# tohtsky/myFM

Measured on AMD Instinct MI355X. Metric: Gibbs iterations/sec (rank=32), higher is better.
Workload: dtype f64

## Files before the change

myfm_amd/csrc/mfm_hip.hip:

```cpp
#include <algorithm>
#include <cerrno>
#include <chrono>
#include <cmath>
#include <cstdio>
#include <cstring>
#include <map>
#include <memory>
#include <mutex>
#include <string>
#include <thread>
#include <type_traits>
#include <vector>

#include <fcntl.h>
#include <sys/file.h>
#include <sys/stat.h>
#include <unistd.h>

#include <hipcub/hipcub.hpp>

#include "mfm_common.hpp"
#include "mfm_kernels.hpp"
#include "mfm_plan.hpp"
#include "mfm_res_plan.hpp"
// ... 68 lines not shown
    d.claimed += want;
    return true;
  }
  void release(int device, int n) {
    if (n <= 0) return;
    std::lock_guard<std::mutex> g(m);
    Dev &d = dev[key_of(device)];
    d.claimed = std::max(0, d.claimed - n);
    if (d.claimed == 0 && d.lock_fd >= 0) {
      ::flock(d.lock_fd, LOCK_UN);
      ::close(d.lock_fd);
      d.lock_fd = -1;
    }
  }
};
}

struct mfm_ctx;
namespace mfm {
static void materialize_e(::mfm_ctx *c);
enum class EWhere : uint8_t { Rows, Slots, SlotsWithSums, Cell, Dropped };
enum class VPath : uint8_t { Deferred, Generic, QFree, Split, SplitFused, TwoField, ShardedSplit, ShardedTwoField, Cell };
enum class ResState : uint8_t { Off, Refused, AwaitingPeers, Live };
}
using namespace mfm;

struct mfm_ctx {
  int device = 0;
  hipStream_t stream = nullptr;
  bool own_stream = false;
  std::string err;
  bool finalized = false;

  HostCsr hX;
  bool main_set = false, hX_valid = false;
  const HostCsr &host_main() {
    if (main_set && !hX_valid) {
      hX = X.download();
      hX_valid = true;
    }
    return hX;
  }
  std::vector<double> hy;
  struct HostBlock {
    HostCsr X;
    std::unique_ptr<int32_t[]> map;
  };
  std::vector<HostBlock> hblocks;
  std::vector<int32_t> hgroup;
  std::vector<int32_t> hlevels;
  int32_t G = 0;

  int64_t N = 0, D0 = 0, D = 0;
  int K = 0, KS = 0;
  DevSparse X;
  StepPlan plan_V, plan_W;
  LongScratch ls;
  Comm comm;
  int64_t row_offset = 0;
  std::vector<std::unique_ptr<DevBlock>> blocks;
  DevBuf<double> y;
  DevBuf<double2> eq_;
  double2 *eq_raw() const { return eq_.p; }
  double2 *eq_rows() {
    mfm::materialize_e(this);
    return eq_.p;
  }
  EWhere e_where = EWhere::Rows;
  bool e_slot_order() const { return e_where == EWhere::Slots || e_where == EWhere::SlotsWithSums; }
  struct ResidentE {
    bool load_slots, no_store;
  };
  ResidentE e_for_resident(bool with_w, int f_begin, int f_end) const {
    return {e_slot_order(), with_w && e_recomputable && e_is_residual && f_begin == 0 && f_end == K};
  }
  void e_left_by_resident(const ResidentE &r) { e_where = r.no_store ? EWhere::Dropped : EWhere::Slots; }
  DevBuf<int32_t> group;
  DevBuf<int32_t> feat_sorted;
  DevBuf<int64_t> group_ptr;

  double w0 = 0;
  DevBuf<double> w, V, Vt;

  DevBuf<double> z;
  DevBuf<double> lam, mu;
  DevBuf<double2> red_partial;
  DevBuf<double2> red_out;
  DevBuf<double> scratch_n;
  DevBuf<double2> gs_partial;
  DevBuf<double2> hs_out;
  DevBuf<double> hs_mu;
  int gs_chunks = 1;
  DevBuf<double> ec, qc;
  VPath v_path = VPath::Generic;
  bool two_field() const { return v_path == VPath::TwoField || v_path == VPath::ShardedTwoField; }
  ResPlan res;
  ResState res_state = ResState::Off;
  bool resident_V() const { return res_state == ResState::Live; }
  std::vector<DevBuf<int32_t>> pre_maps;
  bool e_recomputable = false;
  bool e_is_residual = false;
  int res_plan_cus = 0;
  void ensure_main_plans();
  CellPlan cell;
  bool cell_w = false;
  int q_stale_factor = -1;
  BlockOverflow gather_overflow;
  DevBuf<double> wv_pack, zw_host;
  DevBuf<double> hyp, hyp_in, hyp_ng;
  std::vector<double> hyp_ng_host;
  hipEvent_t hyp_ev = nullptr;
  const double *w0_dev = nullptr;
  std::vector<double> hs_stage;
  bool res_fills_device = false;
  int res_claim = 0;
  DevBuf<double> sync_mask;
  PinnedRing ring;
  double2 *h_red = nullptr;
  size_t h_red_cap = 0;
  Timing timing;

  struct RngEngine {
    bool seeded = false, programmed = false;
    hipStream_t stream = nullptr;
    DevBuf<RngState> state, state_next;
    DevBuf<uint32_t> raw;
    DevBuf<uint32_t> jump;
    uint64_t need_gen = 0;
    int par_wgs = 1;
    int par_blocks = 0;
    DevBuf<uint32_t> starts;
    uint64_t mask = 0, need = 0;
    DevBuf<RngOp> ops;
    int n_ops = 0;
    int64_t n_hv = 0, n_zw = 0, n_zv = 0;
    struct Slot {
      DevBuf<double> hv, zw, zv;
      double *h_hv = nullptr;
      hipEvent_t ready = nullptr, free_ev = nullptr;
      bool free_valid = false;
    } slot[3];
    static constexpr int N_SLOTS = 3;
    hipEvent_t gate = nullptr;
    int pending_slot = -1, pending_op = 0;
    bool latent_pending = false;
    hipEvent_t latent_ev = nullptr;
    DevBuf<uint32_t> host_win;
    int64_t produced = 0, acquired = 0;
    int current = -1;
    std::vector<RngOp> h_ops;
    DevBuf<double> cand;
    DevBuf<unsigned long long> masks;
    DevBuf<int> counts;
    DevBuf<NormScratch> nscratch;
    static constexpr int64_t WIDE_COUNT = 262144;
    static int64_t attempts_for(int64_t count) {
      double a = (double)count * (4.0 / 3.14159265358979) * 1.01 + 8.0 * std::sqrt((double)count + 1.0) + 4096.0;
      int64_t n = (int64_t)a;
      return (n + NORM_CHUNK - 1) / NORM_CHUNK * NORM_CHUNK;
    }
    ~RngEngine() {
      for (auto &sl : slot) {
        if (sl.h_hv) (void)hipHostFree(sl.h_hv);
        if (sl.ready) (void)hipEventDestroy(sl.ready);
        if (sl.free_ev) (void)hipEventDestroy(sl.free_ev);
      }
      if (gate) (void)hipEventDestroy(gate);
      if (latent_ev) (void)hipEventDestroy(latent_ev);
      if (stream) (void)hipStreamDestroy(stream);
    }
  } rng;

  std::unique_ptr<LatentEngine> latent;
  LatentStats latent_stats;
  DevBuf<int32_t> latent_order;

  struct OGroup {
    int n_class = 0;
    int64_t n_rows = 0;
    DevBuf<int32_t> rows;
  };
  std::vector<std::unique_ptr<OGroup>> ogroups;
  int opartial_cmax = 0;
  DevBuf<double> oacc;

  DevBuf<double> opartial;

  ~mfm_ctx() {
    drop_resident();
    if (h_red) (void)hipHostFree(h_red);
    if (own_stream && stream) (void)hipStreamDestroy(stream);
  }
  void use_device() { MFM_HIP_CHECK(hipSetDevice(device)); }
  void drop_resident() {
    for (void *m : res.peer_mapped) (void)hipIpcCloseMemHandle(m);
    res.peer_mapped.clear();
    res_state = ResState::Off;
    res.peers_model = false;
    if (res_claim) ResidentBudget::get().release(device, res_claim);
    res_claim = 0;
    res_fills_device = false;
  }
  void check_coresident(int flag) {
    if (flag == 0) return;
    (void)hipMemsetAsync(ls.error.p, 0, sizeof(int), stream);
    (void)hipStreamSynchronize(stream);
    const bool had = resident_V();
    drop_resident();
    throw Error(MFM_ERR_RUNTIME,
                std::string("co-resident workgroups timed out waiting for each other (long-column sweep / conflict-batched chain / "
                            "resident latent sweep): the state of this fit is invalid") +
                    (flag == 2 ? " [a peer rank's sums did not arrive inside the row-sharded persistent sweep]" : "") +
                    (had ? "; the persistent sweep is switched off for this context" : ""));
  }
  void sync_and_check() {
    if (!ls.error.p) {
      MFM_HIP_CHECK(hipStreamSynchronize(stream));
      return;
    }
    double2 *h = readback(1);
    *(int *)h = 0;
    MFM_HIP_CHECK(hipMemcpyAsync(h, ls.error.p, sizeof(int), hipMemcpyDeviceToHost, stream));
    MFM_HIP_CHECK(hipStreamSynchronize(stream));
    check_coresident(*(const int *)h);
  }
  void need_final() const {
    if (!finalized) throw Error(MFM_ERR_RUNTIME, "mfm_finalize has not been called");
  }
  double2 *readback(size_t n) {
    if (h_red_cap < n) {
      if (h_red) MFM_HIP_CHECK(hipHostFree(h_red));
      h_red = nullptr;
      MFM_HIP_CHECK(hipHostMalloc((void **)&h_red, n * sizeof(double2), hipHostMallocDefault));
      h_red_cap = n;
    }
    return h_red;
  }
};

#define MFM_TRY(ctx) \
  try {              \
    (ctx)->use_device();
#define MFM_CATCH(ctx)                 \
  return MFM_OK;                       \
  }                                    \
  catch (const mfm::Error &ex) {       \
    (ctx)->err = ex.what();            \
    return ex.code;                    \
  }                                    \
  catch (const std::bad_alloc &) {     \
    (ctx)->err = "host out of memory"; \
    return MFM_ERR_RUNTIME;            \
  }                                    \
  catch (const std::exception &ex) {   \
    (ctx)->err = ex.what();            \
    return MFM_ERR_RUNTIME;            \
  }

namespace mfm {

static void fill_gather_args(std::vector<std::unique_ptr<DevBlock>> &blocks, BlockGatherArgs &g, BlockOverflow &ov, PinnedRing &ring,
                             hipStream_t s) {
  std::memset(&g, 0, sizeof(g));
  g.n_blocks = (int)blocks.size();
  std::vector<const int32_t *> xm;
  std::vector<const double *> xr;
  std::vector<int> xs;
  for (size_t b = 0; b < blocks.size(); b++) {
    const int32_t *m = blocks[b]->map.p;
    const double *r = blocks[b]->qc.p ? blocks[b]->qc.p : blocks[b]->rec.p;
    const int st = blocks[b]->qc.p ? 1 : BLOCK_REC;
    if (b < (size_t)MAX_BLOCKS) {
      g.map[b] = m;
      g.rec[b] = r;
      g.stride[b] = st;
    } else {
      xm.push_back(m);
      xr.push_back(r);
      xs.push_back(st);
    }
  }
  BlockOverflow::put(ov.map, xm, ring, s);
  BlockOverflow::put(ov.p0, xr, ring, s);
  BlockOverflow::put(ov.stride, xs, ring, s);
  g.xmap = ov.map.p;
  g.xrec = ov.p0.p;
  g.xstride = ov.stride.p;
}

static bool qbuild_by_rows(const mfm_ctx *c) { return c->X.avg_row_nnz <= 16.0; }
static void launch_qbuild(mfm_ctx *c, const double *vf, DevBlock *pending = nullptr) {
  if (c->N == 0) return;
  hipStream_t s = c->stream;
  BlockGatherArgs g;
  fill_gather_args(c->blocks, g, const_cast<mfm_ctx *>(c)->gather_overflow, const_cast<mfm_ctx *>(c)->ring, s);
  TimedLaunch t(c->timing, s, KC_QBUILD, 12.0 * c->X.nnz + 8.0 * c->N + 8.0 * c->D0 + 12.0 * c->N * g.n_blocks);
  if (qbuild_by_rows(c)) {
    const bool ell = c->X.ell_width >= 0;
    dim3 grid(cdiv(c->N, WG)), block(WG);
#define MFM_QB(U, E) \
  hipLaunchKernelGGL((k_qbuild_rows<U, E>), grid, block, 0, s, c->X.rowptr.p, c->X.colidx.p, c->X.rval.p, vf, c->eq_rows(), c->N, \
                     (int)c->X.ell_width, g, pending ? pending->map.p : (const int32_t *)nullptr,                          \
                     pending ? pending->q_saved.p : (const double2 *)nullptr)
    if (c->X.unit) {
      if (ell) MFM_QB(true, true); else MFM_QB(true, false);
    } else {
      if (ell) MFM_QB(false, true); else MFM_QB(false, false);
// ... 1750 lines not shown
    a.r_val = c->X.rval.p;
    a.r_ell = (int)c->X.ell_width;
    a.state = c->ec.p;
    if (c->v_path != VPath::QFree) {
      a.state2 = c->qc.p;
      a.aos = c->eq_rows();
    }
    return a;
  };
  const bool unit = c->X.unit;
  switch (c->v_path) {
    case VPath::QFree:
      hipLaunchKernelGGL(k_e_pack, dim3(cdiv(c->N, 256)), dim3(256), 0, s, c->eq_rows(), c->ec.p, c->N);
      for (int f = f_begin; f < f_end; f++) run_plan_qfree(s, c->timing, c->plan_V, args(f), c->ls, kcv, unit);
      hipLaunchKernelGGL(k_e_unpack, dim3(cdiv(c->N, 256)), dim3(256), 0, s, c->eq_rows(), c->ec.p, c->N);
      break;
    case VPath::ShardedTwoField:
    case VPath::ShardedSplit: {
      if (c->v_path == VPath::ShardedTwoField) {
        if (unit)
          run_sweep_mf<true>(s, c->timing, c->plan_V, args, f_begin, f_end, c->ls, kcv, &c->comm);
        else
          run_sweep_mf<false>(s, c->timing, c->plan_V, args, f_begin, f_end, c->ls, kcv, &c->comm);
      } else if (c->plan_V.steps.size() > 2) {
        if (unit)
          run_sweep_soa_multi<true>(s, c->timing, c->plan_V, args, f_begin, f_end, c->ls, kcv, &c->comm);
        else
          run_sweep_soa_multi<false>(s, c->timing, c->plan_V, args, f_begin, f_end, c->ls, kcv, &c->comm);
      } else if (unit) {
        run_sweep_soa_sharded<true>(s, c->timing, c->plan_V, args, f_begin, f_end, c->ls, kcv, c->comm);
      } else {
        run_sweep_soa_sharded<false>(s, c->timing, c->plan_V, args, f_begin, f_end, c->ls, kcv, c->comm);
      }
      sync_model_sharded(c, false, f_begin, f_end);
      break;
    }
    case VPath::TwoField:
    case VPath::SplitFused:
    case VPath::Split:
      if (c->v_path == VPath::TwoField) {
        if (unit)
          run_sweep_mf<true>(s, c->timing, c->plan_V, args, f_begin, f_end, c->ls, kcv);
        else
          run_sweep_mf<false>(s, c->timing, c->plan_V, args, f_begin, f_end, c->ls, kcv);
      } else if (unit)
        run_sweep_soa<true>(s, c->timing, c->plan_V, args, f_begin, f_end, c->ls, kcv, c->v_path == VPath::SplitFused);
      else
        run_sweep_soa<false>(s, c->timing, c->plan_V, args, f_begin, f_end, c->ls, kcv, c->v_path == VPath::SplitFused);
      if (!c->plan_V.steps.back().par.tiled)
        hipLaunchKernelGGL(k_e_unpack, dim3(cdiv(c->N, 256)), dim3(256), 0, s, c->eq_rows(), c->ec.p, c->N);
      break;
    case VPath::Cell:
      run_sweep_cell(c, f_begin, f_end, zbase, alpha);
      return MFM_OK;
    case VPath::Generic:
    case VPath::Deferred:
      sweep_V_generic(c, f_begin, f_end, zbase, alpha, kcv);
      return MFM_OK;
  }
  c->q_stale_factor = f_end - 1;
  MFM_HIP_CHECK(hipGetLastError());
  MFM_CATCH(ctx)
}

int mfm_update_e_regression(mfm_ctx *ctx) {
  MFM_TRY(ctx)
  ctx->need_final();
  score_train(ctx, true);
  MFM_CATCH(ctx)
}

int mfm_score_train(mfm_ctx *ctx) {
  MFM_TRY(ctx)
  ctx->need_final();
  score_train(ctx, false);
  MFM_CATCH(ctx)
}

int mfm_rng_seed_mt19937(mfm_ctx *ctx, const uint32_t *state624, int32_t position) {
  MFM_TRY(ctx)
  auto &r = ctx->rng;
  if (position < 0 || position > MT_N) throw Error(MFM_ERR_INVALID, "mt19937 position out of range");
  if (!r.stream) {
    int lo = 0, hi = 0;
    MFM_HIP_CHECK(hipDeviceGetStreamPriorityRange(&lo, &hi));
    MFM_HIP_CHECK(hipStreamCreateWithPriority(&r.stream, hipStreamNonBlocking, hi));
  }
  MFM_HIP_CHECK(hipStreamSynchronize(r.stream));
  RngState h;
  std::memset(&h, 0, sizeof(h));
  h.mt_pos = position;
  std::memcpy(h.mt, state624, sizeof(uint32_t) * MT_N);
  r.state.alloc(1);
  MFM_HIP_CHECK(hipMemcpy(r.state.p, &h, sizeof(h), hipMemcpyHostToDevice));
  r.seeded = true;
  r.produced = r.acquired = 0;
  r.current = -1;
  r.pending_slot = -1;
  for (auto &sl : r.slot) sl.free_valid = false;
  MFM_CATCH(ctx)
}

int mfm_rng_set_program(mfm_ctx *ctx, const mfm_rng_op *ops, int32_t n_ops) {
  MFM_TRY(ctx)
  auto &r = ctx->rng;
  if (!r.seeded) throw Error(MFM_ERR_RUNTIME, "mfm_rng_seed_mt19937 has not been called");
  if (r.produced != r.acquired) throw Error(MFM_ERR_RUNTIME, "cannot change the draw program while a set is in flight");
  MFM_HIP_CHECK(hipStreamSynchronize(r.stream));
  std::vector<RngOp> h((size_t)n_ops);
  int64_t n_dest[3] = {0, 0, 0};
  double normals = 0, gammas = 0;
  int n_normal_ops = 0;
  int64_t latent_rows = 0;
  int n_kept = 0;
  for (int k = 0; k < n_ops; k++) {
    const mfm_rng_op &o = ops[k];
    if (o.kind == MFM_RNG_LATENT) {
      if (o.count < 0) throw Error(MFM_ERR_INVALID, "bad rng op");
      latent_rows += o.count;
      continue;
    }
    const int i = n_kept++;
    if (o.kind != MFM_RNG_NORMALS && o.kind != MFM_RNG_GAMMA) throw Error(MFM_ERR_INVALID, "bad rng op kind");
    if (o.dest < 0 || o.dest > 2 || o.count < 0 || o.offset < 0) throw Error(MFM_ERR_INVALID, "bad rng op");
    if (o.kind == MFM_RNG_GAMMA && !(o.shape > 0)) throw Error(MFM_ERR_INVALID, "gamma shape must be positive");
    h[i].kind = o.kind;
    h[i].dest = o.dest;
    h[i].count = o.kind == MFM_RNG_GAMMA ? 1 : o.count;
    h[i].offset = o.offset;
    h[i].shape = o.shape;
    n_dest[o.dest] = std::max(n_dest[o.dest], o.offset + h[i].count);
    if (o.kind == MFM_RNG_GAMMA)
      gammas += 1;
    else {
      normals += (double)o.count;
      n_normal_ops++;
    }
  }
  h.resize((size_t)n_kept);
  n_ops = n_kept;
  r.n_hv = n_dest[0];
  r.n_zw = n_dest[1];
  r.n_zv = n_dest[2];
  r.ops.upload(h);
  r.h_ops = h;
  r.n_ops = n_ops;
  {
    int64_t amax = 0;
    for (auto &o : h)
      if (o.kind == MFM_RNG_NORMALS && o.count > 16384) amax = std::max(amax, mfm_ctx::RngEngine::attempts_for(o.count));
    r.cand.alloc((size_t)std::max<int64_t>(amax, 1));
    r.masks.alloc((size_t)std::max<int64_t>(amax / 64, 1));
    r.counts.alloc((size_t)std::max<int64_t>(amax / NORM_CHUNK, 1));
    r.nscratch.alloc(1);
  }
  const double per_normal = 4.0 * 4.0 / 3.14159265358979;
  r.need = (uint64_t)(normals * per_normal * 1.02 + 6.0 * 2.4 * std::sqrt(normals + 1.0) + gammas * 4096.0 +
                      4.0 * RNG_ATT * RNG_CONSUME_THREADS * (n_normal_ops + 1) + 65536.0);
  if (latent_rows > 0) r.need += (uint64_t)(4.0 * (1.6 * (double)latent_rows + 6.0 * std::sqrt((double)latent_rows) + 1024.0));
  for (auto &o : h)
    if (o.kind == MFM_RNG_NORMALS && o.count > 16384)
      r.need += (uint64_t)(4 * (mfm_ctx::RngEngine::attempts_for(o.count) - (int64_t)((double)o.count * 1.2732)));
  r.par_wgs = 1;
  r.need_gen = r.need;
  {
    const int64_t blocks1 = (int64_t)(r.need / MT_N) + 2;
    if (blocks1 > MT_PAR_BLOCKS) {
      r.need_gen = r.need * (uint64_t)(latent_rows > (1 << 22) ? 2 : mt_gen_batch((double)r.need));
      const int64_t blocks = (int64_t)(r.need_gen / MT_N) + 2;
      if (r.par_blocks <= 0) r.par_blocks = mt_par_blocks_for(blocks);
      const int wgs = (int)((blocks + r.par_blocks - 1) / r.par_blocks);
      std::vector<uint32_t> tab;
      if (mtjump::JumpCache::inst().get(r.par_blocks, wgs - 1, tab)) {
        r.jump.upload(tab);
        r.state_next.alloc(1);
        r.par_wgs = wgs;
        r.starts.alloc((size_t)wgs * MT_N);
        MFM_HIP_CHECK(hipFuncSetAttribute((const void *)k_mt_generate_par<0>, hipFuncAttributeMaxDynamicSharedMemorySize,
                                          (int)((MT_JUMP_SPAN * MT_N + 2 * (MT_N + 1)) * sizeof(uint32_t))));
        MFM_HIP_CHECK(hipFuncSetAttribute((const void *)k_mt_generate_par<1>, hipFuncAttributeMaxDynamicSharedMemorySize,
                                          (int)((MT_JUMP_SPAN * MT_N + 2 * (MT_N + 1)) * sizeof(uint32_t))));
      }
    }
  }
  uint64_t cap = 1;
  while (cap < r.need_gen + r.need + 2 * MT_N) cap <<= 1;
  r.raw.alloc((size_t)cap);
  r.mask = cap - 1;
  for (auto &sl : r.slot) {
    sl.hv.alloc((size_t)std::max<int64_t>(r.n_hv, 1));
    sl.zw.alloc((size_t)std::max<int64_t>(r.n_zw, 1));
    sl.zv.alloc((size_t)std::max<int64_t>(r.n_zv, 1));
    if (sl.h_hv) MFM_HIP_CHECK(hipHostFree(sl.h_hv));
    sl.h_hv = nullptr;
    MFM_HIP_CHECK(hipHostMalloc((void **)&sl.h_hv, ((size_t)r.n_hv + 4) * sizeof(double), hipHostMallocDefault));
    if (!sl.ready) MFM_HIP_CHECK(hipEventCreateWithFlags(&sl.ready, hipEventDisableTiming));
    if (!sl.free_ev) MFM_HIP_CHECK(hipEventCreateWithFlags(&sl.free_ev, hipEventDisableTiming));
    sl.free_valid = false;
  }
  r.programmed = true;
  MFM_CATCH(ctx)
}

static int rng_enqueue_ops(mfm_ctx *ctx, mfm_ctx::RngEngine::Slot &sl, int first, bool stop_at_wide) {
  auto &r = ctx->rng;
  hipStream_t s = r.stream;
  int i = first;
  while (i < r.n_ops) {
    int j = i;
    while (j < r.n_ops && !(r.h_ops[j].kind == MFM_RNG_NORMALS && r.h_ops[j].count > 16384)) j++;
    if (j > i)
      hipLaunchKernelGGL(k_rng_consume, dim3(1), dim3(RNG_CONSUME_THREADS), 0, s, r.state.p, r.raw.p, r.mask, r.ops.p, i, j,
                         sl.hv.p, sl.zw.p, sl.zv.p);
    if (j < r.n_ops) {
      const RngOp &o = r.h_ops[j];
      if (stop_at_wide && o.count > mfm_ctx::RngEngine::WIDE_COUNT) {
        MFM_HIP_CHECK(hipGetLastError());
        return j;
      }
      const int64_t A = mfm_ctx::RngEngine::attempts_for(o.count);
      const int n_chunks = (int)(A / NORM_CHUNK);
      double *dst = (o.dest == 0 ? sl.hv.p : (o.dest == 1 ? sl.zw.p : sl.zv.p)) + o.offset;
      hipLaunchKernelGGL(k_norm_eval, dim3(n_chunks), dim3(256), 0, s, r.state.p, r.raw.p, r.mask, r.cand.p, r.masks.p,
                         r.counts.p);
      hipLaunchKernelGGL(k_norm_scan, dim3(1), dim3(1024), 0, s, r.state.p, r.counts.p, n_chunks, o.count, r.nscratch.p);
      hipLaunchKernelGGL(k_norm_scatter, dim3(n_chunks), dim3(256), 0, s, r.state.p, r.cand.p, r.masks.p, r.counts.p, o.count,
                         r.nscratch.p, dst);
      j++;
    }
    i = j;
  }
  MFM_HIP_CHECK(hipGetLastError());
  if (r.n_hv)
    MFM_HIP_CHECK(hipMemcpyAsync(sl.h_hv, sl.hv.p, (size_t)r.n_hv * sizeof(double), hipMemcpyDeviceToHost, s));
  MFM_HIP_CHECK(hipMemcpyAsync(sl.h_hv + r.n_hv, r.state.p, 3 * sizeof(double), hipMemcpyDeviceToHost, s));
  MFM_HIP_CHECK(hipEventRecord(sl.ready, s));
  return r.n_ops;
}

static void rng_finish_pending(mfm_ctx *ctx, bool gated) {
  auto &r = ctx->rng;
  if (r.pending_slot < 0) return;
  if (gated) {
    if (!r.gate) MFM_HIP_CHECK(hipEventCreateWithFlags(&r.gate, hipEventDisableTiming));
    MFM_HIP_CHECK(hipEventRecord(r.gate, ctx->stream));
    MFM_HIP_CHECK(hipStreamWaitEvent(r.stream, r.gate, 0));
  }
  const int slot = r.pending_slot;
  r.pending_slot = -1;
  rng_enqueue_ops(ctx, r.slot[slot], r.pending_op, false);
}

int mfm_rng_prefetch(mfm_ctx *ctx) {
  MFM_TRY(ctx)
  auto &r = ctx->rng;
  if (!r.programmed) throw Error(MFM_ERR_RUNTIME, "mfm_rng_set_program has not been called");
  if (r.produced - r.acquired >= (r.current >= 0 ? mfm_ctx::RngEngine::N_SLOTS - 1 : mfm_ctx::RngEngine::N_SLOTS))
    throw Error(MFM_ERR_RUNTIME, "every random set is in use (one acquired, the others in flight): acquire the next one first");
  const bool gated = ctx->resident_V() && ctx->res_fills_device;
  rng_finish_pending(ctx, gated);
  auto &sl = r.slot[r.produced % mfm_ctx::RngEngine::N_SLOTS];
  hipStream_t s = r.stream;
  const bool two_parts = gated && r.produced - r.acquired >= 1;
  if (gated && !two_parts) {
    if (!r.gate) MFM_HIP_CHECK(hipEventCreateWithFlags(&r.gate, hipEventDisableTiming));
    MFM_HIP_CHECK(hipEventRecord(r.gate, ctx->stream));
    MFM_HIP_CHECK(hipStreamWaitEvent(s, r.gate, 0));
  }
  if (sl.free_valid) MFM_HIP_CHECK(hipStreamWaitEvent(s, sl.free_ev, 0));
  if (r.latent_pending) {
    if (!r.latent_ev) MFM_HIP_CHECK(hipEventCreateWithFlags(&r.latent_ev, hipEventDisableTiming));
    MFM_HIP_CHECK(hipEventRecord(r.latent_ev, ctx->stream));
    MFM_HIP_CHECK(hipStreamWaitEvent(s, r.latent_ev, 0));
    r.latent_pending = false;
  }
  if (r.par_wgs > 1) {
    hipLaunchKernelGGL(k_mt_generate_par<1>, dim3(r.par_wgs), dim3(MT_GEN_THREADS),
                       (MT_JUMP_SPAN * MT_N + 2 * (MT_N + 1)) * sizeof(uint32_t), s, r.state.p, r.state_next.p, r.raw.p, r.mask,
                       r.need_gen, r.jump.p, r.par_blocks, r.starts.p, r.need);
    hipLaunchKernelGGL(k_mt_generate_par<2>, dim3(r.par_wgs), dim3(MT_GEN_THREADS), 2 * (MT_N + 1) * sizeof(uint32_t), s,
                       r.state.p, r.state_next.p, r.raw.p, r.mask, r.need_gen, r.jump.p, r.par_blocks, r.starts.p, r.need);
    hipLaunchKernelGGL(k_mt_commit, dim3(1), dim3(MT_GEN_THREADS), 0, s, r.state.p, r.state_next.p);
  } else {
    hipLaunchKernelGGL(k_mt_generate, dim3(1), dim3(MT_GEN_THREADS), 0, s, r.state.p, r.raw.p, r.mask, r.need);
  }
  const int slot_idx = (int)(r.produced % mfm_ctx::RngEngine::N_SLOTS);
  const int next_op = rng_enqueue_ops(ctx, sl, 0, two_parts);
  if (next_op < r.n_ops) {
    r.pending_slot = slot_idx;
    r.pending_op = next_op;
  }
  r.produced++;
  MFM_CATCH(ctx)
}

int mfm_rng_acquire(mfm_ctx *ctx, double *hyper_variates, int64_t n_hyper_variates) {
  MFM_TRY(ctx)
  auto &r = ctx->rng;
  if (r.produced <= r.acquired) throw Error(MFM_ERR_RUNTIME, "no prefetched random set: call mfm_rng_prefetch first");
  if (n_hyper_variates != r.n_hv) throw Error(MFM_ERR_INVALID, "hyper variate count does not match the draw program");
  if (r.current >= 0) {
    auto &prev = r.slot[r.current];
    MFM_HIP_CHECK(hipEventRecord(prev.free_ev, ctx->stream));
    prev.free_valid = true;
  }
  if (r.pending_slot == (int)(r.acquired % mfm_ctx::RngEngine::N_SLOTS)) rng_finish_pending(ctx, false);
  auto &sl = r.slot[r.acquired % mfm_ctx::RngEngine::N_SLOTS];
  MFM_HIP_CHECK(hipEventSynchronize(sl.ready));
  RngState hdr;
  std::memcpy(&hdr, sl.h_hv + r.n_hv, 3 * sizeof(double));
  if (hdr.error) throw Error(MFM_ERR_RUNTIME, "device random stream underflow (generated range exhausted)");
  if (r.n_hv) std::memcpy(hyper_variates, sl.h_hv, (size_t)r.n_hv * sizeof(double));
  r.current = (int)(r.acquired % mfm_ctx::RngEngine::N_SLOTS);
  r.acquired++;
  MFM_CATCH(ctx)
}

int mfm_rng_get_z(mfm_ctx *ctx, double *zw, double *zv) {
  MFM_TRY(ctx)
  auto &r = ctx->rng;
  if (r.current < 0) throw Error(MFM_ERR_RUNTIME, "no acquired random set");
  auto &sl = r.slot[r.current];
  if (zw && r.n_zw) MFM_HIP_CHECK(hipMemcpy(zw, sl.zw.p, (size_t)r.n_zw * sizeof(double), hipMemcpyDeviceToHost));
  if (zv && r.n_zv) MFM_HIP_CHECK(hipMemcpy(zv, sl.zv.p, (size_t)r.n_zv * sizeof(double), hipMemcpyDeviceToHost));
  MFM_CATCH(ctx)
}

int mfm_timing_enable(mfm_ctx *ctx, int on) {
  MFM_TRY(ctx)
  if (!on) ctx->timing.resolve();
  ctx->timing.on = on != 0;
  MFM_CATCH(ctx)
}

int mfm_timing_select(mfm_ctx *ctx, int32_t kernel_class) {
  MFM_TRY(ctx)
  if (kernel_class >= KC_N) throw Error(MFM_ERR_INVALID, "kernel class index out of range");
  ctx->timing.only = kernel_class < 0 ? -1 : kernel_class;
  MFM_CATCH(ctx)
}
int mfm_timing_reset(mfm_ctx *ctx) {
  MFM_TRY(ctx)
  MFM_HIP_CHECK(hipStreamSynchronize(ctx->stream));
  ctx->timing.reset();
  MFM_CATCH(ctx)
}
int mfm_timing_n_classes(void) { return KC_N; }
const char *mfm_timing_class_name(int cls) { return (cls >= 0 && cls < KC_N) ? kKernelClassNames[cls] : ""; }
int mfm_timing_get(mfm_ctx *ctx, int cls, double *ms_total, int64_t *launches, double *alg_bytes_total) {
  MFM_TRY(ctx)
  if (cls < 0 || cls >= KC_N) throw Error(MFM_ERR_INVALID, "bad kernel class");
  MFM_HIP_CHECK(hipStreamSynchronize(ctx->stream));
  ctx->timing.resolve();
  *ms_total = ctx->timing.ms[cls];
  *launches = ctx->timing.launches[cls];
  *alg_bytes_total = ctx->timing.bytes[cls];
  MFM_CATCH(ctx)
}

int mfm_host_column_levels(int64_t n_rows, int64_t n_cols, const int64_t *indptr, const int32_t *indices, int32_t *level,
                           int32_t *n_levels) {
  try {
    HostCsr X;
    X.rows = n_rows;
    X.cols = n_cols;
    X.ptr.assign(indptr, indptr + n_rows + 1);
    X.idx.assign(indices, indices + indptr[n_rows]);
    X.val.assign((size_t)indptr[n_rows], 1.0);
    HostCsr Xt = transpose_host(X);
    std::vector<int32_t> lv;
    *n_levels = column_levels(Xt, lv);
    std::copy(lv.begin(), lv.end(), level);
    return MFM_OK;
  } catch (const std::exception &ex) {
    g_global_error = ex.what();
    return MFM_ERR_RUNTIME;
  }
}

}
// ... 12 lines not shown
```

myfm_amd/csrc/mfm_rng.hpp:

```cpp
#pragma once
#include <hip/hip_runtime.h>
#include <stdint.h>

#include <algorithm>
#include <cstdlib>

#include "mfm_rng_state.hpp"

namespace mfm {

#ifndef MFM_RNG_CONSUME_THREADS
#define MFM_RNG_CONSUME_THREADS 1024
#endif
constexpr int RNG_CONSUME_THREADS = MFM_RNG_CONSUME_THREADS;
constexpr int RNG_ATT = 4;
#ifndef MFM_RNG_SPEC
#define MFM_RNG_SPEC 16
#endif

struct RngOp {
  int32_t kind;
  int32_t dest;
  int64_t count;
  int64_t offset;
// ... 264 lines not shown
        saved = x * mult;
        have_saved = 1;
        n = y * mult;
      }
      asm volatile("" : "+v"(have_saved));
      n = n * 1.0 + 0.0;
      v = 1.0 + a2 * n;
      if (v > 0.0 || g.past) break;
    }
    v = v * v * v;
    u = g.uniform();
    const bool again = u > 1.0 - 0.0331 * n * n * n * n && (log(u) > (0.5 * n * n + a1 * (1.0 - v + log(v))));
    if (!again || g.past) break;
  }
  if (alpha == malpha) return a1 * v;
  do u = g.uniform();
  while (u == 0.0 && !g.past);
  return pow(u, 1.0 / alpha) * a1 * v;
}

__global__ __launch_bounds__(RNG_CONSUME_THREADS) void k_rng_consume(RngState *__restrict__ st,
                                                                     const uint32_t *__restrict__ raw, uint64_t mask,
                                                                     const RngOp *__restrict__ ops, int op_begin,
                                                                     int op_end, double *__restrict__ hv,
                                                                     double *__restrict__ zw, double *__restrict__ zv) {
  constexpr int NW = RNG_CONSUME_THREADS / 64;
  constexpr int WIN = 8192;
  __shared__ int s_tot[RNG_ATT][NW];
  __shared__ unsigned long long s_p;
  __shared__ int s_kstar;
  __shared__ uint32_t s_win[WIN];
  __shared__ double s_gval[NW][64];
  __shared__ int s_gend[NW][64];
  const int tid = threadIdx.x, lane = tid & 63, wid = tid >> 6;
  uint64_t p = st->p_cons;
  const uint64_t p_gen_at_start = st->p_gen;
  uint64_t wbase = 0;
  uint32_t wlen = 0;
  for (int oi = op_begin; oi < op_end; oi++) {
    const RngOp op = ops[oi];
    double *dst = (op.dest == 0 ? hv : (op.dest == 1 ? zw : zv)) + op.offset;
    if (op.kind == 1) {
      int n_run = 1;
      while (oi + n_run < op_end && ops[oi + n_run].kind == 1) n_run++;
      int done_ops = 0;
      while (done_ops < n_run) {
        if (p < wbase || p + 2048 > wbase + wlen) {
          __syncthreads();
          for (int i = tid; i < WIN; i += RNG_CONSUME_THREADS) s_win[i] = mt_temper(raw[(p + (uint64_t)i) & mask]);
          wbase = p;
          wlen = WIN;
          __syncthreads();
        }
        const int batch = min(MFM_RNG_SPEC < NW ? MFM_RNG_SPEC : NW, n_run - done_ops);
        if (wid < batch && (MFM_RNG_SPEC > 1 || lane == 0)) {
          const RngOp oj = ops[oi + done_ops + wid];
          RawReader g{raw, mask, p + (uint64_t)(6 * wid + 2 * lane), s_win, wbase, wlen, p_gen_at_start};
          s_gval[wid][lane] = gamma_unit(g, oj.shape);
          s_gend[wid][lane] = g.past ? -1 : (int)(g.p - p);
        }
        __syncthreads();
        if (tid == 0) {
          int pos = 0, j = 0;
          for (; j < batch; j++) {
            const int l2 = pos - 6 * j;
            if (l2 < 0 || l2 >= 128) break;
            const RngOp oj = ops[oi + done_ops + j];
            double *dj = (oj.dest == 0 ? hv : (oj.dest == 1 ? zw : zv)) + oj.offset;
            dj[0] = s_gval[j][l2 >> 1];
            if (s_gend[j][l2 >> 1] < 0) {
              st->error = 1;
              pos += 6;
            } else {
              pos = s_gend[j][l2 >> 1];
            }
          }
          s_p = p + (uint64_t)pos;
          s_kstar = j;
        }
        __syncthreads();
        p = s_p;
        done_ops += s_kstar;
        __syncthreads();
      }
      oi += n_run - 1;
      continue;
    }
    int64_t done = 0;
    while (done < op.count) {
      bool acc[RNG_ATT];
      double yv[RNG_ATT], r2v[RNG_ATT];
      unsigned long long bal[RNG_ATT];
#pragma unroll
      for (int r = 0; r < RNG_ATT; r++) {
        const uint64_t base = p + 4ull * (uint64_t)(r * RNG_CONSUME_THREADS + tid);
        const uint32_t u0 = mt_temper(raw[(base + 0) & mask]), u1 = mt_temper(raw[(base + 1) & mask]);
        const uint32_t u2 = mt_temper(raw[(base + 2) & mask]), u3 = mt_temper(raw[(base + 3) & mask]);
        const double x = 2.0 * canonical(u0, u1) - 1.0;
        const double y = 2.0 * canonical(u2, u3) - 1.0;
        const double r2 = x * x + y * y;
        acc[r] = !(r2 > 1.0 || r2 == 0.0);
        yv[r] = y;
        r2v[r] = r2;
        bal[r] = __ballot(acc[r]);
        if (lane == 0) s_tot[r][wid] = __popcll(bal[r]);
      }
      __syncthreads();
      const int64_t needed = op.count - done;
      int64_t run = 0;
      int64_t total = 0;
      int rank[RNG_ATT];
#pragma unroll
      for (int r = 0; r < RNG_ATT; r++) {
        int before = 0, tot = 0;
#pragma unroll
        for (int w = 0; w < NW; w++) {
          const int t = s_tot[r][w];
          before += (w < wid) ? t : 0;
          tot += t;
        }
        rank[r] = (int)run + before + __popcll(bal[r] & ((1ull << lane) - 1ull));
        run += tot;
      }
      total = run;
      const bool last_batch = total >= needed;
#pragma unroll
      for (int r = 0; r < RNG_ATT; r++) {
        if (acc[r] && rank[r] < needed) {
          const double mult = sqrt(-2 * log(r2v[r]) / r2v[r]);
          dst[done + rank[r]] = (yv[r] * mult) * 1.0 + 0.0;
          if (last_batch && rank[r] == needed - 1) s_kstar = r * RNG_CONSUME_THREADS + tid;
        }
      }
      __syncthreads();
      if (last_batch) {
        p += 4ull * (uint64_t)(s_kstar + 1);
        done = op.count;
      } else {
        p += 4ull * (uint64_t)(RNG_ATT * RNG_CONSUME_THREADS);
        done += total;
      }
      __syncthreads();
    }
  }
  if (tid == 0) {
    st->p_cons = p;
    if (p > st->p_gen) st->error = 1;
  }
}


constexpr int NORM_CHUNK = 1024;

struct NormScratch {
  unsigned long long p_base;
  int32_t insufficient;
  int32_t pad;
};

__global__ __launch_bounds__(256) void k_norm_eval(const RngState *__restrict__ st, const uint32_t *__restrict__ raw,
                                                   uint64_t mask, double *__restrict__ cand,
                                                   unsigned long long *__restrict__ masks, int *__restrict__ counts) {
  __shared__ int s_cnt[4];
  const uint64_t p = st->p_cons;
  const int tid = threadIdx.x, lane = tid & 63, wid = tid >> 6;
  int cnt = 0;
#pragma unroll
  for (int r = 0; r < 4; r++) {
    const int64_t a = (int64_t)blockIdx.x * NORM_CHUNK + r * 256 + tid;
    const uint64_t base = p + 4ull * (uint64_t)a;
    const uint32_t u0 = mt_temper(raw[(base + 0) & mask]), u1 = mt_temper(raw[(base + 1) & mask]);
    const uint32_t u2 = mt_temper(raw[(base + 2) & mask]), u3 = mt_temper(raw[(base + 3) & mask]);
    const double x = 2.0 * canonical(u0, u1) - 1.0;
    const double y = 2.0 * canonical(u2, u3) - 1.0;
    const double r2 = x * x + y * y;
    const bool acc = !(r2 > 1.0 || r2 == 0.0);
    if (acc) {
      const double mult = sqrt(-2 * log(r2) / r2);
      cand[a] = (y * mult) * 1.0 + 0.0;
    }
    const unsigned long long b = __ballot(acc);
    if (lane == 0) {
      masks[a >> 6] = b;
      cnt += __popcll(b);
    }
  }
  if (lane == 0) s_cnt[wid] = cnt;
  __syncthreads();
  if (tid == 0) counts[blockIdx.x] = s_cnt[0] + s_cnt[1] + s_cnt[2] + s_cnt[3];
}

__global__ __launch_bounds__(1024) void k_norm_scan(const RngState *__restrict__ st, int *__restrict__ counts, int n_chunks,
                                                    int64_t count, NormScratch *__restrict__ ns) {
  __shared__ int s_w[16];
  __shared__ int s_carry;
  const int tid = threadIdx.x, lane = tid & 63, wid = tid >> 6;
  if (tid == 0) s_carry = 0;
  __syncthreads();
  for (int base = 0; base < n_chunks; base += 1024) {
    const int i = base + tid;
    const int v = i < n_chunks ? counts[i] : 0;
    int incl = v;
#pragma unroll
    for (int d = 1; d < 64; d <<= 1) {
      const int o = __shfl_up(incl, d, 64);
      if (lane >= d) incl += o;
    }
    if (lane == 63) s_w[wid] = incl;
    __syncthreads();
    int woff = 0;
    for (int w = 0; w < wid; w++) woff += s_w[w];
    const int carry = s_carry;
    if (i < n_chunks) counts[i] = carry + woff + incl - v;
    __syncthreads();
    if (tid == 1023) s_carry = carry + woff + incl;
    __syncthreads();
  }
  if (tid == 0) {
    ns->p_base = st->p_cons;
    ns->insufficient = (int64_t)s_carry < count ? 1 : 0;
  }
}

__global__ __launch_bounds__(256) void k_norm_scatter(RngState *__restrict__ st, const double *__restrict__ cand,
                                                      const unsigned long long *__restrict__ masks,
                                                      const int *__restrict__ offs, int64_t count,
                                                      const NormScratch *__restrict__ ns, double *__restrict__ dst) {
  const int tid = threadIdx.x, lane = tid & 63, wid = tid >> 6;
  const unsigned long long *m = masks + (int64_t)blockIdx.x * (NORM_CHUNK / 64);
  int64_t before = offs[blockIdx.x];
#pragma unroll
  for (int r = 0; r < 4; r++) {
    int wbefore = 0;
    for (int w = 0; w < 4; w++) {
      const int c = __popcll(m[r * 4 + w]);
      if (w < wid) wbefore += c;
    }
    const unsigned long long b = m[r * 4 + wid];
    const bool acc = (b >> lane) & 1ull;
    const int64_t rank = before + wbefore + __popcll(b & ((1ull << lane) - 1ull));
    const int64_t a = (int64_t)blockIdx.x * NORM_CHUNK + r * 256 + tid;
    if (acc && rank < count) {
      dst[rank] = cand[a];
      if (rank == count - 1) {
        st->p_cons = ns->p_base + 4ull * (unsigned long long)(a + 1);
        if (ns->insufficient) st->error = 1;
      }
    }
    for (int w = 0; w < 4; w++) before += __popcll(m[r * 4 + w]);
  }
  if (blockIdx.x == 0 && tid == 0 && ns->insufficient) st->error = 1;
}

}
```

Before: 380.3.

## Fold normal-sampler prefix scan into scatter kernel, dropping separate scan launch

The single-block scan kernel and its scratch buffer are removed. Each scatter block now computes its own exclusive offset by summing the per-chunk acceptance counts of all earlier blocks, using a strided loop plus a wave reduction. The last block detects an insufficient accepted count and sets the error flag. The aim is to remove one serialized kernel launch, and its one-block bottleneck, per wide normal op. In exchange, the total counts read grows quadratically with the number of chunks.

Result: no change. 382.7, median of 4 (+0.6%).

```diff
diff --git a/myfm_amd/csrc/mfm_hip.hip b/myfm_amd/csrc/mfm_hip.hip
--- a/myfm_amd/csrc/mfm_hip.hip
+++ b/myfm_amd/csrc/mfm_hip.hip
@@ -244,7 +244,6 @@
     DevBuf<double> cand;
     DevBuf<unsigned long long> masks;
     DevBuf<int> counts;
-    DevBuf<NormScratch> nscratch;
     static constexpr int64_t WIDE_COUNT = 262144;
     static int64_t attempts_for(int64_t count) {
       double a = (double)count * (4.0 / 3.14159265358979) * 1.01 + 8.0 * std::sqrt((double)count + 1.0) + 4096.0;
@@ -2301,7 +2300,6 @@
     r.cand.alloc((size_t)std::max<int64_t>(amax, 1));
     r.masks.alloc((size_t)std::max<int64_t>(amax / 64, 1));
     r.counts.alloc((size_t)std::max<int64_t>(amax / NORM_CHUNK, 1));
-    r.nscratch.alloc(1);
   }
   const double per_normal = 4.0 * 4.0 / 3.14159265358979;
   r.need = (uint64_t)(normals * per_normal * 1.02 + 6.0 * 2.4 * std::sqrt(normals + 1.0) + gammas * 4096.0 +
@@ -2372,9 +2370,8 @@
       double *dst = (o.dest == 0 ? sl.hv.p : (o.dest == 1 ? sl.zw.p : sl.zv.p)) + o.offset;
       hipLaunchKernelGGL(k_norm_eval, dim3(n_chunks), dim3(256), 0, s, r.state.p, r.raw.p, r.mask, r.cand.p, r.masks.p,
                          r.counts.p);
-      hipLaunchKernelGGL(k_norm_scan, dim3(1), dim3(1024), 0, s, r.state.p, r.counts.p, n_chunks, o.count, r.nscratch.p);
-      hipLaunchKernelGGL(k_norm_scatter, dim3(n_chunks), dim3(256), 0, s, r.state.p, r.cand.p, r.masks.p, r.counts.p, o.count,
-                         r.nscratch.p, dst);
+      hipLaunchKernelGGL(k_norm_scatter, dim3(n_chunks), dim3(256), 0, s, r.state.p, r.cand.p, r.masks.p, r.counts.p, n_chunks,
+                         o.count, dst);
       j++;
     }
     i = j;
diff --git a/myfm_amd/csrc/mfm_rng.hpp b/myfm_amd/csrc/mfm_rng.hpp
--- a/myfm_amd/csrc/mfm_rng.hpp
+++ b/myfm_amd/csrc/mfm_rng.hpp
@@ -440,12 +440,6 @@
 
 constexpr int NORM_CHUNK = 1024;
 
-struct NormScratch {
-  unsigned long long p_base;
-  int32_t insufficient;
-  int32_t pad;
-};
-
 __global__ __launch_bounds__(256) void k_norm_eval(const RngState *__restrict__ st, const uint32_t *__restrict__ raw,
                                                    uint64_t mask, double *__restrict__ cand,
                                                    unsigned long long *__restrict__ masks, int *__restrict__ counts) {
@@ -478,45 +472,20 @@
   if (tid == 0) counts[blockIdx.x] = s_cnt[0] + s_cnt[1] + s_cnt[2] + s_cnt[3];
 }
 
-__global__ __launch_bounds__(1024) void k_norm_scan(const RngState *__restrict__ st, int *__restrict__ counts, int n_chunks,
-                                                    int64_t count, NormScratch *__restrict__ ns) {
-  __shared__ int s_w[16];
-  __shared__ int s_carry;
-  const int tid = threadIdx.x, lane = tid & 63, wid = tid >> 6;
-  if (tid == 0) s_carry = 0;
-  __syncthreads();
-  for (int base = 0; base < n_chunks; base += 1024) {
-    const int i = base + tid;
-    const int v = i < n_chunks ? counts[i] : 0;
-    int incl = v;
-#pragma unroll
-    for (int d = 1; d < 64; d <<= 1) {
-      const int o = __shfl_up(incl, d, 64);
-      if (lane >= d) incl += o;
-    }
-    if (lane == 63) s_w[wid] = incl;
-    __syncthreads();
-    int woff = 0;
-    for (int w = 0; w < wid; w++) woff += s_w[w];
-    const int carry = s_carry;
-    if (i < n_chunks) counts[i] = carry + woff + incl - v;
-    __syncthreads();
-    if (tid == 1023) s_carry = carry + woff + incl;
-    __syncthreads();
-  }
-  if (tid == 0) {
-    ns->p_base = st->p_cons;
-    ns->insufficient = (int64_t)s_carry < count ? 1 : 0;
-  }
-}
-
 __global__ __launch_bounds__(256) void k_norm_scatter(RngState *__restrict__ st, const double *__restrict__ cand,
                                                       const unsigned long long *__restrict__ masks,
-                                                      const int *__restrict__ offs, int64_t count,
-                                                      const NormScratch *__restrict__ ns, double *__restrict__ dst) {
+                                                      const int *__restrict__ counts, int n_chunks, int64_t count,
+                                                      double *__restrict__ dst) {
+  __shared__ int s_w[4];
   const int tid = threadIdx.x, lane = tid & 63, wid = tid >> 6;
+  int part = 0;
+  for (int i = tid; i < (int)blockIdx.x; i += 256) part += counts[i];
+#pragma unroll
+  for (int d = 32; d > 0; d >>= 1) part += __shfl_xor(part, d, 64);
+  if (lane == 0) s_w[wid] = part;
+  __syncthreads();
   const unsigned long long *m = masks + (int64_t)blockIdx.x * (NORM_CHUNK / 64);
-  int64_t before = offs[blockIdx.x];
+  int64_t before = s_w[0] + s_w[1] + s_w[2] + s_w[3];
 #pragma unroll
   for (int r = 0; r < 4; r++) {
     int wbefore = 0;
@@ -530,14 +499,11 @@
     const int64_t a = (int64_t)blockIdx.x * NORM_CHUNK + r * 256 + tid;
     if (acc && rank < count) {
       dst[rank] = cand[a];
-      if (rank == count - 1) {
-        st->p_cons = ns->p_base + 4ull * (unsigned long long)(a + 1);
-        if (ns->insufficient) st->error = 1;
-      }
+      if (rank == count - 1) st->p_cons = st->p_cons + 4ull * (unsigned long long)(a + 1);
     }
     for (int w = 0; w < 4; w++) before += __popcll(m[r * 4 + w]);
   }
-  if (blockIdx.x == 0 && tid == 0 && ns->insufficient) st->error = 1;
-}
-
-}
+  if ((int)blockIdx.x == n_chunks - 1 && tid == 0 && before < count) st->error = 1;
+}
+
+}
```
